# NyanCAD/Cadnip.jl

Hardware: AMD Instinct MI355X
Metric: newton_iters_per_sec (higher is better)
Workload: dtype f64; 1 GPU; gf180 DFF transient 0-700 ns (synthetic sp_mos1 level-1 card, 30 MOSFETs, n=235, nnz=1090), 4096 Vdd x temp corner instances per GPU (state resident in HBM; one 8-instance workgroup per CU in flight, the rest handed out by the kernel's instance queue); step = DC init + full transient of the batch; instances_per_gpu=4096, instances_total=4096, fused=2, newton_mode=1, launches_last_step=5120, accepted_last_step=6078488, rejected_last_step=692364

## Files before the change

### cadnip.jl_amd/csrc/devices.hpp

```cpp
#pragma once
#include <hip/hip_runtime.h>
#include <math.h>
#include "../../include/cadnip_hip.h"

namespace cadnip {

#define CADNIP_CHARGE_SCALE 1e12

#ifdef CADNIP_TRACE
static __device__ unsigned long long g_trace_sum[64], g_trace_cnt[64];
static __device__ int g_trace_wave;
__shared__ unsigned long long g_trace_last;
#define CADNIP_TRACE_FINE(id) (((id) >= 8 && (id) <= 15) || (id) >= 18 || (id) == 0 || (id) == 2)
#define CADNIP_TRACE_POINT(id)                                                                          \
  do {                                                                                                  \
    if ((CADNIP_TRACE + 0 >= 2 || !CADNIP_TRACE_FINE(id)) && blockIdx.x == 0 && (int)(threadIdx.x >> 6) == g_trace_wave) { \
      unsigned long long _t = clock64();                                                                \
      if ((threadIdx.x & 63) == 0) {                                                                    \
        atomicAdd(&g_trace_sum[id], _t - g_trace_last); atomicAdd(&g_trace_cnt[id], 1ull); g_trace_last = _t; \
      }                                                                                                 \
    }                                                                                                   \
  } while (0)
#define CADNIP_TRACE_USE(x) asm volatile("" ::"v"(x))
#elif defined(CADNIP_MARKS)
#define CADNIP_TRACE_POINT(id) asm volatile("; @@MARK " #id)
#define CADNIP_TRACE_USE(x) do {} while (0)
#else
#define CADNIP_TRACE_POINT(id) do {} while (0)
#define CADNIP_TRACE_USE(x) do {} while (0)
#endif

__device__ __forceinline__ double dpp_pair_swap(double v) {
  int lo = __double2loint(v), hi = __double2hiint(v);
  lo = __builtin_amdgcn_update_dpp(0, lo, 0xB1, 0xF, 0xF, false);
  hi = __builtin_amdgcn_update_dpp(0, hi, 0xB1, 0xF, 0xF, false);
  return __hiloint2double(hi, lo);
}

template <class NodeT> struct DevCtxT {
  const NodeT* __restrict__ nodes;
  const int* __restrict__ ipar;
  const double* __restrict__ par;
  const double* __restrict__ wave;
  int count;
// ... 525 lines not shown
  {
    const bool fwd = o_vds >= 0;
    const double q_vgs = fwd ? vgs : vgd + (vgs - vgd), q_vgd = fwd ? vgs - (vgs - vgd) : vgd, q_vds = vgs - vgd;
    const bool c1 = fabs(fwd ? vgs - o_vgs : vgd - vgdo) <= 0.4, c2 = fabs(q_vds - o_vds) <= 0.4;
    const bool c3 = q_vds >= 0 ? !(fabs(vbs - o_vbs) > (vt + vt)) : !(fabs(vbd - o_vbd) > (vt + vt));
    if (__all(c1 && c2 && c3)) {
      double r_vgs = q_vgs, r_vds = q_vds, r_vbs, r_vbd;
      (void)q_vgd;
      if (r_vds >= 0) { r_vbs = vbs; r_vbd = r_vbs - r_vds; }
      else { r_vbd = vbd; r_vbs = r_vbd + r_vds; }
      if (d.initjct) { r_vbs = -1; r_vgs = type * par_of(d, M1_TVTO); r_vds = 0; r_vbd = r_vbs - r_vds; }
      w_gs = type * r_vgs; w_ds = type * r_vds; w_bs = type * r_vbs; w_bd = type * r_vbd;
      return;
    }
  }
  int omode = o_vds >= 0 ? 1 : -1;
  double osel = omode == 1 ? o_vbs : o_vbd, osarg;
  if (osel <= 0) osarg = sqrt(tPhi - osel);
  else { osarg = sqrt(tPhi); osarg = osarg - o_vbs / (osarg + osarg); osarg = fmax(0.0, osarg); }
  double o_von = (tVbi * type) + gamma * osarg;
  double von = type * o_von;
  if (o_vds >= 0) {
    vgs = m1_fetlim(vgs, o_vgs, von);
    vds = vgs - vgd;
    vds = m1_limvds(vds, o_vds);
    vgd = vgs - vds;
  } else {
    vgd = m1_fetlim(vgd, vgdo, von);
    vds = vgs - vgd;
    vds = -m1_limvds(-vds, -o_vds);
// ... 466 lines not shown
```

### cadnip.jl_amd/csrc/fused2_kernel.hpp

```cpp
#pragma once
#include <hip/hip_runtime.h>
#include "devices.hpp"
#include "internal.hpp"
#include "tran_ctrl.hpp"
#include "lds_layout.hpp"
#include "src_cache.hpp"

namespace cadnip {

typedef unsigned short u16;
typedef unsigned long long u64;
#define NOPOS 0xFFFFu
#define F2_NCMAX 16
#define F2_JU 18
#define F2_MAX_BLOCKS 32

enum { S_GPOS = 0, S_CDESC, S_BROW, S_NZ, S_ENT, S_TERM, S_LEV, S_QINV, S_NODES, S_ROWOF, S_LOADPOS, S_NSEC };

struct F2Block {
  const int* ipar; const double* par;
  int type, count, n_par, g_base, c_base, b_base, nodes_off, mos1_plain;
  int lds_par;
};

// ... 85 lines not shown
    atomicAdd(&W[tg(gpos[k * count + dev])], v);
  }
  __device__ __forceinline__ void C(int k, double v) const {
    if (!JAC) return;
    if (__builtin_constant_p(v) && v == 0.0) return;
    const u64 d = cdesc[k * count + dev];
    atomicAdd(&W[tg((unsigned)d & 0xFFFFu)], a0 * v);
    if (!DIRECT) atomicAdd(&W[tg((unsigned)(d >> 16) & 0xFFFFu)], v * betas[(unsigned)(d >> 32) & 0xFFFFu]);
  }
  __device__ __forceinline__ void B(int k, double v) const {
    if (DIRECT || (__builtin_constant_p(v) && v == 0.0)) return;
    atomicAdd(&W[tg(brow[k * count + dev])], -v);
  }
  template <int N> __device__ __forceinline__ void Gv(int k0, const double (&v)[N]) const {
    if (!JAC) return;
    unsigned p[N];
#pragma unroll
    for (int i = 0; i < N; ++i) p[i] = gpos[(k0 + i) * count + dev];
#pragma unroll
    for (int i = 0; i < N; ++i) if (!(__builtin_constant_p(v[i]) && v[i] == 0.0)) atomicAdd(&W[tg(p[i])], v[i]);
  }
  template <int N> __device__ __forceinline__ void Gk(const int (&k)[N], const double (&v)[N]) const {
    if (!JAC) return;
    unsigned p[N];
#pragma unroll
    for (int i = 0; i < N; ++i) p[i] = gpos[k[i] * count + dev];
#pragma unroll
    for (int i = 0; i < N; ++i) atomicAdd(&W[tg(p[i])], v[i]);
  }
  template <int N> __device__ __forceinline__ void Cv(int k0, const double (&v)[N]) const {
// ... 14 lines not shown
      }
  }
  template <int N> __device__ __forceinline__ void Bv(int k0, const double (&v)[N]) const {
    if (DIRECT) return;
    unsigned p[N];
#pragma unroll
    for (int i = 0; i < N; ++i) p[i] = brow[(k0 + i) * count + dev];
#pragma unroll
    for (int i = 0; i < N; ++i) if (!(__builtin_constant_p(v[i]) && v[i] == 0.0)) atomicAdd(&W[tg(p[i])], -v[i]);
  }
};

typedef DevCtxT<short> LdsCtx;

struct F2M1ParMem {
  int bi, inst, dev;
  __device__ __forceinline__ double operator()(int k) const {
    const F2ArgsK ka = kargs();
    const F2Block B = load_block(ka->blk, bi);
    return (B.par + (size_t)inst * B.n_par * B.count)[k * B.count + dev];
  }
};

template <bool LEAN, class Out>
__device__ __forceinline__ void dispatch_stamp2(int type, const LdsCtx& d, const double* u, const Out& s, double* lw) {
  if constexpr (LEAN) {
    switch (type) {
      case CADNIP_DEV_RESISTOR: stamp_resistor(d, u, s, lw); break;
      case CADNIP_DEV_CAPACITOR: stamp_capacitor(d, u, s, lw); break;
      case CADNIP_DEV_INDUCTOR: stamp_inductor(d, u, s, lw); break;
      case CADNIP_DEV_VSOURCE: stamp_vsource(d, u, s, lw); break;
      case CADNIP_DEV_ISOURCE: stamp_isource(d, u, s, lw); break;
      case CADNIP_DEV_VCVS: stamp_vcvs(d, u, s, lw); break;
      case CADNIP_DEV_VCCS: stamp_vccs(d, u, s, lw); break;
// ... 83 lines not shown
  __device__ __forceinline__ double h3(int i, int) const { return (kargs()->t.u3 + vo)[i]; }
  __device__ __forceinline__ void set_h3(int i, int, double v) { (kargs()->t.u3 + vo)[i] = v; }
  __device__ __forceinline__ void set_h0(int i, int k, double v) { if (k >= 0) r_u0[k] = v; else p_u0()[i] = v; }
  __device__ __forceinline__ void set_h1(int i, int k, double v) { if (k >= 0) r_u1[k] = v; else p_u1()[i] = v; }
  __device__ __forceinline__ void set_h2(int i, int k, double v) { if (k >= 0) r_u2[k] = v; else p_u2()[i] = v; }
  __device__ __forceinline__ void set_hp(int i, int k, double v) { if (k >= 0) r_up[k] = v; else p_up()[i] = v; }
  __device__ __forceinline__ double atol_of(const TranArgs& a, int i, int k) const { return k >= 0 ? pf_at[k] : a.atol[i]; }
  __device__ __forceinline__ double emask_of(const TranArgs& a, int i, int k) const { return k >= 0 ? pf_em[k] : a.emask[i]; }
};

template <int NC, int MODE>
__device__ __forceinline__ void dense_core_solve(double* W, int dn0, int yc0, int lane, int& bad, bool keep) {
  const int row = lane < NC ? lane : 0;
  double* S = W + dn0 + row * NC;
  double A[NC], rp[NC], bc = W[yc0 + row];
#pragma unroll
  for (int j = 0; j < NC; ++j) A[j] = S[j];
#pragma unroll
  for (int k = 0; k < NC; ++k) {
    const double pkk = readlane_f64(A[k], k);
    if (MODE == 0 && (pkk == 0.0 || !isfinite(pkk))) bad = 1;
    rp[k] = MODE == 0 ? fast_div(1.0, pkk) : pkk;
    const double m = lane > k ? (MODE == 0 ? A[k] * rp[k] : A[k]) : 0.0;
    if (MODE == 0) {
#pragma unroll
      for (int j = k + 1; j < NC; ++j) A[j] = fma(-m, readlane_f64(A[j], k), A[j]);
      if (lane > k) A[k] = m;
    }
    bc = fma(-m, readlane_f64(bc, k), bc);
  }
// ... 41 lines not shown
      const uint4* src = (const uint4*)f.team_desc;
      uint4* dst = (uint4*)L.desc;
      unsigned char* fl = (unsigned char*)(L.desc + f.team_desc_len);
      for (int i = tid; i < f.team_desc_len / 2; i += 64 * WPB) {
        const uint4 d = src[i];
        const StepPredec p = lds_step_predecode(d.x, d.y, d.z, d.w, (unsigned)(f.nnz_lu + n + lane0));
        dst[i] = make_uint4(p.x, p.y, p.z, p.w);
        fl[i] = (unsigned char)p.flags;
      }
    } else {
      const uint2* src = (const uint2*)f.team_desc;
      uint2* dst = (uint2*)L.desc;
      for (int i = tid; i < f.team_desc_len; i += 64 * WPB) dst[i] = src[i];
    }
  }
  __syncthreads();
  const int nW = L.nW;
  double* W = L.W;
  double* us = L.u;
  double* betas = L.beta;
  if (lane0 == 0) { W[nW] = 0.0; W[nW + 1] = 1.0; }
  const int tlo = f.tab_lo;
  const u16* gpos = (const u16*)(tab + (f.off[S_GPOS] - tlo));
  const u64* cdesc = (const u64*)(tab + (f.off[S_CDESC] - tlo));
  const u16* brow = (const u16*)(tab + (f.off[S_BROW] - tlo));
  const u64* nzd = (const u64*)(tab + (LEAN ? 0 : f.off[S_NZ]));
  const u64* laned = (const u64*)(tab + (LEAN ? 0 : f.off[S_ENT]));
  const unsigned* term = tab + (LEAN ? 0 : f.off[S_TERM]);
  typedef const __attribute__((address_space(4))) u64* PassPtr;
  const PassPtr passd = (PassPtr)(const u64*)(f.tab + f.off[S_LEV]);
  const u16* qinv = (const u16*)(tab + (f.off[S_QINV] - tlo));
  const short* nodes = (const short*)(tab + (f.off[S_NODES] - tlo));
  const u16* rowof = (const u16*)(tab + (f.off[S_ROWOF] - tlo));
  unsigned rc_gp[RCQ][2] = {}, rc_row[RCQ] = {}, rc_nd[RCQ] = {}, src_gp[2] = {0, 0}, src_row[2] = {0, 0}, src_nd[2] = {0, 0};
  int rc_count = 0, rc_type = 0, src_count = 0, src_type = 0;
  M1PairView<F2M1ParMem> m1v;
  if constexpr (DIRECT) {
    const unsigned tr = (unsigned)(f.nnz_lu + n + lane0);
    auto row_of = [&](int node) -> unsigned { return node < 0 ? tr : (unsigned)rowof[node]; };
    if (SHAPE ? true : f.rc_blk >= 0) {
      const F2Block B = load_block(f.blk, f.rc_blk);
      rc_count = B.count; rc_type = B.type;
      const short* nd = nodes + B.nodes_off;
#pragma unroll
      for (int q = 0; q < RCQ; ++q) {
        const int dev = lane0 + 64 * q;
        unsigned p[4] = {tr, tr, tr, tr};
        int np = -1, nn = -1;
        if (dev < B.count) {
          np = nd[dev]; nn = nd[B.count + dev];
#pragma unroll
// ... 10 lines not shown
      src_count = B.count; src_type = B.type;
      const short* nd = nodes + B.nodes_off;
      unsigned p[4] = {tr, tr, tr, tr};
      int np = -1, nn = -1, ni = -1;
      if (lane0 < B.count) {
        np = nd[lane0]; nn = nd[B.count + lane0];
        if (SHAPE ? true : B.type == CADNIP_DEV_VSOURCE) {
          ni = nd[2 * B.count + lane0];
#pragma unroll
          for (int k = 0; k < 4; ++k) p[k] = (unsigned)gpos[B.g_base + k * B.count + lane0];
        }
      }
      src_gp[0] = p[0] | p[1] << 16; src_gp[1] = p[2] | p[3] << 16;
      src_row[0] = row_of(np) | row_of(nn) << 16; src_row[1] = row_of(ni);
      src_nd[0] = ((unsigned)np & 0xFFFFu) | ((unsigned)nn & 0xFFFFu) << 16; src_nd[1] = (unsigned)ni & 0xFFFFu;
    }
    if constexpr (SHAPE) {
      const F2Block B = load_block(f.blk, 3 - f.rc_blk - f.src_blk);
      const short* nd = nodes + B.nodes_off;
      const int dv = lane0 >> 1, dev = dv < B.count ? dv : B.count - 1, sd = lane0 & 1;
      const int vdep = B.ipar[dev];
      auto node = [&](int k) -> int { return nd[k * B.count + dev]; };
      auto qnode = [&](int r) -> int { return ((vdep >> r) & 1) ? node(10 + r) : -1; };
      auto opd2 = [&](int na, int nb) -> unsigned { return lds_m1pin_operand(na, f.nnz_lu, n) | lds_m1pin_operand(nb, f.nnz_lu, n) << 16; };
      auto row2 = [&](int na, int nb) -> unsigned { return lds_m1pin_row(rowof, na, tr) | lds_m1pin_row(rowof, nb, tr) << 16; };
#pragma unroll
      for (int j = 0; j < 5; ++j) m1v.opd[j] = opd2(node(2 * j), node(2 * j + 1));
      m1v.opd[5] = opd2(qnode(sd), qnode(2 + sd));
      m1v.row[0] = sd ? row2(node(8), node(9)) : row2(node(6), node(7));
      m1v.row[1] = row2(sd ? node(4) : node(3), node(5));
      m1v.row[2] = row2(qnode(sd), sd ? node(3) : node(1));
      m1v.row[3] = row2(qnode(2 + sd), sd ? node(5) : node(4));
      m1v.initjct = 0;
      m1v.gnd = lds_m1pin_operand(-1, f.nnz_lu, n); m1v.beta = 8u * (unsigned)n;
    }
  }
#ifdef CADNIP_TRACE
  if (blockIdx.x == 0 && tid == 0) g_trace_last = clock64();
#endif
  int inst = blockIdx.x * WPB + w;
  int budget = f.rounds;
  for (;;) {
  StepState st;
  bool have = false;
  while (inst < f.B) {
    const TranStateView sv = state_view<FIXED>();
    if (DC) st.status = __builtin_amdgcn_readfirstlane(sv.status[inst]);
    else { st = load_state(sv, inst); make_uniform(st); }
// ... 42 lines not shown
  double src_val = 0.0, src_t = 0.0;
  bool src_have = false;
  int src_seg = 0;
  for (; budget > 0; --budget) {
    int lane = lane0;
    asm volatile("" : "+v"(lane));
    CADNIP_TRACE_POINT(17);
    bool refresh = true;
    if (mn) {
      refresh = (st.mflags & MN_NEED) || !(st.mflags & MN_VALID) ||
                (st.k == 0 && (st.a0 < 0.6 * st.a0f || st.a0 * 0.6 > st.a0f || (st.mflags >> MN_SINCE_SHIFT) >= 20));
      if (refresh) { st.a0f = st.a0; st.ss = 20.0; st.mflags = MN_VALID | MN_JCUR; st.dsc = 1.0; }
      else st.dsc = st.a0 == st.a0f ? 1.0 : fast_div(2.0, 1.0 + fast_div(st.a0, st.a0f));
    }
    if (refresh) {
      for (int i = lane; i < (nW >> 1); i += 64) ((double2*)W)[i] = make_double2(0.0, 0.0);
    } else if constexpr (FIXED) {
#pragma unroll
      for (int k = 0; k < 5; ++k) { const int i = f.nnz_lu + lane + 64 * k; if (i < nW) W[i] = 0.0; }
    } else {
      for (int i = f.nnz_lu + lane; i < nW; i += 64) W[i] = 0.0;
    }
    CADNIP_WAVE_SYNC();
    CADNIP_TRACE_POINT(0);
    const double tcur = DC ? 0.0 : st.tn, a0 = DC ? 0.0 : st.a0;
    const int dmode = DC ? f.dc_mode : 1, dinit = DC ? dc_first : 0;
    const unsigned trash_w = (unsigned)(f.nnz_lu + n + lane);
    dc_first = 0;
    if constexpr (DIRECT) {
      auto at = [&](unsigned nd16) -> double { const double x = us[nd16 == 0xFFFFu ? 0u : nd16]; return nd16 == 0xFFFFu ? 0.0 : x; };
// ... 4 lines not shown
      };
      if (SHAPE ? true : f.rc_blk >= 0) {
        const bool cap = SHAPE ? true : rc_type == CADNIP_DEV_CAPACITOR;
        double jv[RCQ], cur[RCQ];
#pragma unroll
        for (int q = 0; q < RCQ; ++q) {
          const unsigned np = rc_nd[q] & 0xFFFFu, nn = rc_nd[q] >> 16;
          const double xp = cap ? dat(np) : at(np), xn = cap ? dat(nn) : at(nn);
          jv[q] = cap ? a0 * rc_val[q] : rc_val[q];
          cur[q] = rc_val[q] * (xp - xn);
        }
#pragma unroll
        for (int q = 0; q < RCQ; ++q) {
          if (q == 1 && rc_count <= 64) break;
          if (refresh) {
            atomicAdd(&W[rc_gp[q][0] & 0xFFFFu], jv[q]); atomicAdd(&W[rc_gp[q][0] >> 16], -jv[q]);
            atomicAdd(&W[rc_gp[q][1] & 0xFFFFu], -jv[q]); atomicAdd(&W[rc_gp[q][1] >> 16], jv[q]);
          }
          atomicAdd(&W[rc_row[q] & 0xFFFFu], cur[q]); atomicAdd(&W[rc_row[q] >> 16], -cur[q]);
        }
      }
      CADNIP_TRACE_POINT(14);
      if (SHAPE ? true : f.src_blk >= 0) {
        if (DC || !src_have || tcur != src_t) {
          const int cl = src_cache_lanes(src_count);
          const bool sc = sc_on();
          int miss = 1;
          double cv = 0.0;
          if (sc) {
            const SrcSeg e = src_seg_load((const double*)L.src, cl, lane < cl ? lane : 0);
            miss = src_seg_hit(e, tcur) ? 0 : 1;
            cv = src_seg_value(e, tcur);
          }
          if (wave_any(miss)) {
            const F2Block B = load_block(f.blk, f.src_blk);
            const double* par = B.par + (size_t)inst * B.n_par * B.count;
            LdsCtx d{nodes + B.nodes_off, B.ipar, par, f.wave, B.count, lane < B.count ? lane : 0, tcur, dmode, dinit};
            src_val = source_value(d, par_of(d, 0), par_of(d, 1), &src_seg);
          } else src_val = cv;
          if (sc_on() && miss && lane < cl) {
            const F2ArgsK ka = kargs();
            const F2Block B = load_block(ka->blk, ka->src_blk);
            SrcSeg r = src_seg_never();
            if (B.ipar[lane] == 1) {
              const int len = B.ipar[2 * B.count + lane];
              const double* wv = ka->wave + B.ipar[B.count + lane];
              r = src_seg_refill(1, wv, wv + len, len, src_seg, (B.par + (size_t)inst * B.n_par * B.count)[B.count + lane]);
            }
            src_seg_store(L.src, cl, lane, r);
          }
          src_t = tcur; src_have = true;
        }
        CADNIP_TRACE_USE(src_val);
        CADNIP_TRACE_POINT(15);
        if (SHAPE ? true : src_type == CADNIP_DEV_VSOURCE) {
          const double ui = at(src_nd[1]), vd = at(src_nd[0] & 0xFFFFu) - at(src_nd[0] >> 16) - src_val;
          if (refresh) {
            atomicAdd(&W[src_gp[0] & 0xFFFFu], 1.0); atomicAdd(&W[src_gp[0] >> 16], -1.0);
            atomicAdd(&W[src_gp[1] & 0xFFFFu], 1.0); atomicAdd(&W[src_gp[1] >> 16], -1.0);
          }
          atomicAdd(&W[src_row[0] & 0xFFFFu], ui); atomicAdd(&W[src_row[0] >> 16], -ui);
          atomicAdd(&W[src_row[1]], vd);
        } else {
          atomicAdd(&W[src_row[0] & 0xFFFFu], -src_val); atomicAdd(&W[src_row[0] >> 16], src_val);
        }
      }
      CADNIP_TRACE_POINT(13);
    }
    if constexpr (SHAPE) {
      const int bi = 3 - f.rc_blk - f.src_blk;
      const F2Block B = load_block(f.blk, bi);
      const int side = lane & 1;
      const int dv = lane >> 1;
      const bool valid = dv < B.count;
      const int dev = valid ? dv : B.count - 1;
#pragma unroll
      for (int j = 0; j < 6; ++j) asm volatile("" : "+v"(m1v.opd[j]));
#pragma unroll
      for (int j = 0; j < 4; ++j) asm volatile("" : "+v"(m1v.row[j]));
      m1_pair_each_param(m1v, [](double& x) { asm volatile("" : "+v"(x)); });
      m1v.W = W; m1v.mem = F2M1ParMem{bi, inst, dev};
      if (!refresh) {
        AccumOutT<true, DIRECT, false> s{W, betas, a0, gpos + B.g_base, cdesc + B.c_base, brow + B.b_base, B.count, dev, valid ? 0u : trash_w, us, rowof, trash_w};
        stamp_mos1_pair(m1v, us, s, lw, side, valid);
      } else {
        AccumOutT<true, DIRECT> s{W, betas, a0, gpos + B.g_base, cdesc + B.c_base, brow + B.b_base, B.count, dev, valid ? 0u : trash_w, us, rowof, trash_w};
        stamp_mos1_pair(m1v, us, s, lw, side, valid);
      }
      CADNIP_TRACE_POINT(8);
    }
    if constexpr (!SHAPE)
    for (int bi = 0; bi < f.n_blk; ++bi) {
      if (DIRECT && ((bi == f.rc_blk && rc_count <= 128) || (bi == f.src_blk && src_count <= 64))) continue;
      const F2Block B = load_block(f.blk, bi);
      const double* par = B.par + (size_t)inst * B.n_par * B.count;
      int dev0 = lane;
      if (DIRECT && bi == f.rc_blk) dev0 = lane + 128;
      if (DIRECT && bi == f.src_blk) dev0 = lane + 64;
      if (!DIRECT && bi == f.rc_blk) {
#pragma unroll
        for (int q = 0; q < 2; ++q) {
// ... 159 lines not shown
        double part = fma(a2v, b2v, fma(a1v, b1v, a0v * b0v));
        if (maxlg >= 1) { const double o = dpp_f64<0xB1>(part); part += lg >= 1 ? o : 0.0; }
        if (maxlg >= 2) { const double o = dpp_f64<0x4E>(part); part += lg >= 2 ? o : 0.0; }
        if (maxlg >= 3) { const double o = dpp_f64<0x141>(part); part += lg >= 3 ? o : 0.0; }
        if (maxlg >= 4) { const double o = dpp_f64<0x140>(part); part += lg >= 4 ? o : 0.0; }
        double acc = acc0 - part;
        if (fw >> 31) {
          if (piv == 0.0 || !isfinite(piv)) bad = 1;
          acc = fast_div(acc, piv);
        }
        *((D.x & 0x8000u) ? pp : W + trash_w) = acc;
        D = Dn;
      }
      CADNIP_WAVE_SYNC();
    };
    auto run_steps_pd = [&](const int s_first, const int s_count) {
      if (s_count <= 0) return;
      const uint4* dp = tdesc + (size_t)s_first * 64 + lane;
      const unsigned char* fp = tflag + (size_t)s_first * 64 + lane;
      char* const Wb = (char*)W;
      uint4 D = dp[0];
      unsigned F = fp[0];
      for (int si = 0; si < s_count; ++si) {
        double* const pp = (double*)(Wb + (D.x & 0xFFFFu));
        const double piv = *(const double*)(Wb + (D.x >> 16));
        const double a0v = *(const double*)(Wb + (D.y & 0xFFFFu)), b0v = *(const double*)(Wb + (D.y >> 16));
        const double a1v = *(const double*)(Wb + (D.z & 0xFFFFu)), b1v = *(const double*)(Wb + (D.z >> 16));
        const double a2v = *(const double*)(Wb + (D.w & 0xFFFFu)), b2v = *(const double*)(Wb + (D.w >> 16));
        const double acc0 = *pp;
        const uint4 Dn = dp[(size_t)(si + 1) * 64];
        const unsigned Fn = fp[(size_t)(si + 1) * 64];
        const unsigned fs = __builtin_amdgcn_readfirstlane(F), maxlg = fs & 7u;
        double part = fma(a2v, b2v, fma(a1v, b1v, a0v * b0v));
        if (maxlg >= 1) { const double o = dpp_f64<0xB1>(part); part += F >= 16u ? o : 0.0; }
        if (maxlg >= 2) { const double o = dpp_f64<0x4E>(part); part += F >= 32u ? o : 0.0; }
        if (maxlg >= 3) { const double o = dpp_f64<0x141>(part); part += F >= 48u ? o : 0.0; }
        if (maxlg >= 4) { const double o = dpp_f64<0x140>(part); part += F >= 64u ? o : 0.0; }
        double acc = acc0 - part;
        if (fs & 8u) {
          if (piv == 0.0 || !isfinite(piv)) bad = 1;
          acc = fast_div(acc, piv);
        }
        *pp = acc;
        D = Dn; F = Fn;
      }
      CADNIP_WAVE_SYNC();
    };
    auto solve_steps = [&](const int s_first, const int s_count) {
      if (predec) run_steps_pd(s_first, s_count); else run_steps(s_first, s_count);
    };
    if constexpr (LEAN) {
      solve_steps(refresh ? 0 : f.ts_pre + f.ts_post, refresh ? f.ts_pre : f.ts_fwd);
    } else {
      if (refresh) run_passes(0, f.n_pre);
      else run_passes(f.n_pre + f.n_post, f.n_fwd);
    }
    CADNIP_TRACE_POINT(4);
    if constexpr (FIXED) {
      const int yc0 = f.nnz_lu + n - 8;
      if (refresh) dense_core_solve<8, 0>(W, f.dn0, yc0, lane, bad, true);
      else dense_core_solve<8, 1>(W, f.dn0, yc0, lane, bad, false);
      CADNIP_WAVE_SYNC();
    } else if (f.nc > 0) {
      const int yc0 = f.nnz_lu + n - f.nc;
      if (refresh) DENSE_CORE(0, f.nc, W, f.dn0, yc0, lane, bad, mn);
      else if (LEAN && !DC) DENSE_CORE(1, f.nc, W, f.dn0, yc0, lane, bad, false);
      CADNIP_WAVE_SYNC();
    }
    CADNIP_TRACE_POINT(5);
    if constexpr (LEAN) solve_steps(f.ts_pre, f.ts_post); else run_passes(f.n_pre, f.n_post);
    CADNIP_TRACE_POINT(3);
    if (DC) {
      for (int i = lane; i < n; i += 64) { const double dd = W[qinv[i]]; if (!isfinite(dd)) bad = 1; us[i] -= dd; }
      bad = wave_any(bad);
      CADNIP_WAVE_SYNC();
      if (f.dc_pcnr && a.n_limits > 0) {
        __builtin_amdgcn_fence(__ATOMIC_ACQ_REL, "workgroup");
        for (int i = n - a.n_limits + lane; i < n; i += 64) us[i] = lw[i];
      }
      if (bad) st.status = -2; else dc_iters += 1;
    } else {
      tran_update_body(a, vec, st, inst, lane, bad);
      make_uniform(st);
    }
    CADNIP_WAVE_SYNC();
// ... 50 lines not shown
```

### cadnip.jl_amd/csrc/lds_layout.hpp

```cpp
#pragma once
#include <stddef.h>
#include "../../include/cadnip_hip.h"
#ifdef __HIPCC__
#include <type_traits>
#define LDS_HD __host__ __device__ __forceinline__
#else
#define LDS_HD inline
#endif

#define F2_TRASH 64
#define LDS_BUDGET ((size_t)160 * 1024)
#define LDS_OPTIN ((size_t)64 * 1024)

namespace cadnip {

LDS_HD int lds_work_words(int lu_words, int n) { return lu_words + n + F2_TRASH; }
#define LDS_CONSTS 2

struct StepPredec { unsigned x, y, z, w, flags; };
LDS_HD StepPredec lds_step_predecode(unsigned x, unsigned y, unsigned z, unsigned w, unsigned trash_word) {
  StepPredec r;
  r.x = ((x & 0x8000u) ? (x & 0x7FFFu) : trash_word) << 3 | ((x >> 16) & 0x7FFFu) << 19;
  r.y = (y & 0x7FFF7FFFu) << 3; r.z = (z & 0x7FFF7FFFu) << 3; r.w = (w & 0x7FFF7FFFu) << 3;
  const unsigned lg = (x >> 31) | ((y >> 14) & 2u) | ((y >> 29) & 4u);
// ... 6 lines not shown
                        int use_pcnr, bool enabled) {
  return tran && lean && newton_mode == 1 && step_predec && src_words > 0 && n <= 256 && nc == 8 && max_order <= 2 && step_rule == 0 &&
         use_pcnr == 0 && enabled;
}
LDS_HD bool f2_shape_ok(bool fixed, int n_blk, int src_type, int src_count, int rc_type, int rc_count, int dev_type, int dev_plain, int dev_count,
                        bool enabled) {
  return fixed && n_blk == 3 && src_type == CADNIP_DEV_VSOURCE && src_count <= 64 && rc_type == CADNIP_DEV_CAPACITOR && rc_count <= 64 &&
         dev_type == CADNIP_DEV_MOS1 && dev_plain != 0 && dev_count <= 32 && enabled;
}
LDS_HD bool lds_m1pin_ok(int lu_words, int n) { return lds_work_words(lu_words, n) + LDS_CONSTS + n <= 8192; }
LDS_HD unsigned lds_m1pin_operand(int node, int lu_words, int n) {
  const int nW = lds_work_words(lu_words, n);
  return (unsigned)(node < 0 ? nW : nW + LDS_CONSTS + node) << 3;
}
template <class T> LDS_HD unsigned lds_m1pin_row(const T* rowof, int node, unsigned trash_word) { return node < 0 ? trash_word : (unsigned)rowof[node]; }
LDS_HD int lds_sweep_desc_words(int desc_len, bool predec) { return desc_len + (predec ? desc_len / 16 : 0); }

template <class P> struct LdsSweep { P desc, W, u, beta, end; int nW, per; P src; };
template <class P> LDS_HD LdsSweep<P> lds_sweep(P base, int tab_len, int desc_len, int lu_words, int n, int w, int wpb, int src_words = 0) {
  LdsSweep<P> L;
  L.nW = lds_work_words(lu_words, n);
  L.per = L.nW + LDS_CONSTS + 2 * n + src_words;
  L.desc = base + tab_len / 2;
  L.W = L.desc + desc_len + (size_t)w * L.per;
  L.u = L.W + L.nW + LDS_CONSTS; L.beta = L.u + n; L.src = L.beta + n;
  L.end = L.desc + desc_len + (size_t)wpb * L.per;
  return L;
}

template <class P> struct LdsTeam { P W, red, u, beta, par, desc, priv, end; int nW; };
// ... 56 lines not shown
```

### cadnip.jl_amd/csrc/tran_ctrl.hpp

```cpp
#pragma once
#include <hip/hip_runtime.h>
#include <math.h>

namespace cadnip {

#define CADNIP_WAVE_SYNC() do { __builtin_amdgcn_fence(__ATOMIC_ACQ_REL, "wavefront"); __builtin_amdgcn_wave_barrier(); } while (0)

template <int CTRL> __device__ __forceinline__ double dpp_f64(double v) {
  int lo = __double2loint(v), hi = __double2hiint(v);
  lo = __builtin_amdgcn_update_dpp(0, lo, CTRL, 0xF, 0xF, true);
  hi = __builtin_amdgcn_update_dpp(0, hi, CTRL, 0xF, 0xF, true);
  return __hiloint2double(hi, lo);
}
__device__ __forceinline__ double group_sum16(double v, int width) {
  if (width >= 2) v += dpp_f64<0xB1>(v);
  if (width >= 4) v += dpp_f64<0x4E>(v);
  if (width >= 8) v += dpp_f64<0x141>(v);
  if (width >= 16) v += dpp_f64<0x140>(v);
  return v;
}
__device__ __forceinline__ double readlane_f64(double v, int l) {
  return __hiloint2double(__builtin_amdgcn_readlane(__double2hiint(v), l), __builtin_amdgcn_readlane(__double2loint(v), l));
}
__device__ __forceinline__ double wave_sum(double v) {
// ... 16 lines not shown
  int e;
  double m = frexp(x, &e);
  const int q = (e >= 0 ? e : e - 2) / 3;
  m = ldexp(m, e - 3 * q);
  double y = fma(m, -0.17, 1.18);
#pragma unroll
  for (int it = 0; it < 4; ++it) {
    const double y3 = (y * y) * y;
    y = (y * fma(-m, y3, 4.0)) * (1.0 / 3.0);
  }
  return ldexp(y, -q);
}

#ifndef CADNIP_TRACE_POINT
#define CADNIP_TRACE_POINT(id) do {} while (0)
#endif
struct TranArgs {
  double *u, *du, *delta, *limit_w, *tcur, *gamma;
  int *active, *flags;
  double *t, *h, *hprev, *hpp; int *nhist, *order, *k, *status, *bp_idx, *save_idx; long long* cnt;
  double *u0, *u1, *u2, *up, *beta;
  const double *atol, *emask, *breaks, *save_t; const int* obs; double* out; int* nactive;
  int B, n, n_limits, n_break, n_save, n_obs, n_err;
  double t0, t1, reltol, h0, hmin, hmax, newton_tol;
  int max_newton, max_order, use_pcnr;
  int newton_mode;
  double *mn_a0f, *mn_ss, *mn_dnp; int* mn_flags;
  int step_rule;
  double *u3, *hp3;
};
// ... 142 lines not shown
  }
}

template <class V>
__device__ inline void prepare_step(const TranArgs& a, V& v, StepState& s, int tid, double t, double h, int nhist, double hprev, double hpp) {
  const int n = a.n;
  double tstop = a.t1;
  if (s.t_break < tstop) tstop = s.t_break;
  double rem = tstop - t, tn;
  if (h >= rem * (1.0 - 1e-9)) { h = rem; tn = tstop; }
  else if (2.0 * h > rem) { h = 0.5 * rem; tn = t + h; }
  else tn = t + h;
  int ord;
  double a0;
  if (nhist <= 1) {
    ord = 1; a0 = fast_div(1.0, h);
    each_elem<V>(n, tid, [&](int i, int k) { double p = v.h0(i, k); v.set_hp(i, k, p); v.set_u(i, p); double b = fast_div(-p, h); v.set_beta(i, b); v.set_du(i, a0 * p + b); });
  } else if (nhist == 2 || a.max_order < 2) {
    ord = 1; a0 = fast_div(1.0, h);
    double w = fast_div(h, hprev);
    each_elem<V>(n, tid, [&](int i, int k) {
      double x0 = v.h0(i, k);
      double p = x0 + w * (x0 - v.h1(i, k));
      v.set_hp(i, k, p); v.set_u(i, p);
      double b = fast_div(-x0, h);
      v.set_beta(i, b); v.set_du(i, a0 * p + b);
    });
  } else if (nhist >= 4 && (!V::FIXED && a.max_order >= 3)) {
    ord = 3;
    const double hr = s.hp3;
    const double d1 = h, d2 = h + hprev, d3 = d2 + hpp, s12 = hprev + hpp;
    a0 = (fast_div(1.0, d1) + fast_div(1.0, d2)) + fast_div(1.0, d3);
    const double a1 = -fast_div(d2 * d3, d1 * (hprev * s12)), a2 = fast_div(d1 * d3, d2 * (hprev * hpp)), a3 = -fast_div(d1 * d2, d3 * (s12 * hpp));
// ... 22 lines not shown
      double x0 = v.h0(i, k), xm1 = v.h1(i, k);
      double p = L0 * x0 + L1 * xm1 + L2 * v.h2(i, k);
      v.set_hp(i, k, p); v.set_u(i, p);
      double b = a1 * x0 + a2 * xm1;
      v.set_beta(i, b); v.set_du(i, a0 * p + b);
    });
  }
  s.h = h; s.ord = ord; s.k = 0; s.tn = tn; s.a0 = a0;
  s.mflags &= ~MN_JCUR;
}

template <class V>
__device__ inline void save_outputs(const TranArgs& a, V& v, StepState& s, int inst, int tid) {
  const double told = s.t, tn = s.tn, hh = tn - told;
  int si = s.si;
  if (s.t_save <= tn * (1.0 + 1e-15)) v.history_to_memory(a.n, tid);
  while (s.t_save <= tn * (1.0 + 1e-15)) {
    double ts = s.t_save;
    double* o = a.out + ((size_t)inst * a.n_save + si) * a.n_obs;
    if (s.nhist >= 2) {
      double x = ts - told, xa = hh, xc = -s.hprev;
      double La = fast_div((x - 0.0) * (x - xc), (xa - 0.0) * (xa - xc));
      double Lb = fast_div((x - xa) * (x - xc), (0.0 - xa) * (0.0 - xc));
      double Lc = fast_div((x - xa) * (x - 0.0), (xc - xa) * (xc - 0.0));
      for (int j = tid; j < a.n_obs; j += V::NT) { int i = a.obs[j]; o[j] = La * v.get_u(i) + Lb * v.mem_u0(i) + Lc * v.mem_u1(i); }
    } else {
      double sc = fast_div(ts - told, hh);
      for (int j = tid; j < a.n_obs; j += V::NT) { int i = a.obs[j]; double x0 = v.mem_u0(i); o[j] = x0 + sc * (v.get_u(i) - x0); }
    }
    ++si;
    s.t_save = next_save(a, si);
  }
// ... 58 lines not shown
      const int nh_cap = (!V::FIXED && a.max_order >= 3) ? 4 : 3;
      int nh_new = s.nhist + 1 > nh_cap ? nh_cap : s.nhist + 1;
      double hnext;
      if (tested) {
        double fac;
        if (V::FIXED || a.step_rule == 0) {
          fac = errn > 0.0 ? 0.9 * step_root(errn, (V::FIXED ? (s.ord == 1 ? 1 : 2) : s.ord)) : 2.0;
          fac = fmin(2.0, fmax(0.2, fac));
        } else {
          const double eta = errn > 0.0 ? fast_div(1.0, fast_div(1.0, step_root(2.0 * errn, (V::FIXED ? (s.ord == 1 ? 1 : 2) : s.ord))) + 1e-4) : 2.0;
          fac = eta >= 2.0 ? 2.0 : (eta <= 1.0 ? fmax(0.5, fmin(0.9, eta)) : 1.0);
        }
        hnext = h * fac;
      } else hnext = 2.0 * h;
      if (landed) {
        ++s.bp;
        s.t_break = next_break(a, s.bp);
        nh_new = 1;
        double tstop = a.t1;
        if (s.t_break < tstop) tstop = s.t_break;
        hnext = 0.1 * fmin(h, tstop - tn);
      }
      hnext = fmin(hnext, a.hmax);
      s.hp3 = hpp;
      s.t = tn; s.hpp = hprev; s.hprev = h; s.nhist = nh_new;
      s.c_accept += 1;
      s.mflags += 1 << MN_SINCE_SHIFT;
      CADNIP_TRACE_POINT(31);
      if (tn >= a.t1) { s.status = 1; return; }
      if (hnext < a.hmin) hnext = a.hmin;
      grp_sync<V>();
      prepare_step(a, v, s, tid, tn, hnext, nh_new, s.hprev, s.hpp);
      CADNIP_TRACE_POINT(32);
    } else {
      double fac;
      if (V::FIXED || a.step_rule == 0) { fac = 0.9 * step_root(errn, (V::FIXED ? (s.ord == 1 ? 1 : 2) : s.ord)); fac = fmin(0.9, fmax(0.1, fac)); }
      else { fac = fast_div(0.9, fast_div(1.0, step_root(2.0 * errn, (V::FIXED ? (s.ord == 1 ? 1 : 2) : s.ord))) + 1e-4); fac = fmin(0.9, fmax(0.25, fac)); }
      double hn = h * fac;
      s.c_reject += 1;
      if (hn < a.hmin) { s.status = -1; return; }
      grp_sync<V>();
      prepare_step(a, v, s, tid, s.t, hn, s.nhist, hprev, hpp);
    }
  } else {
    if ((V::FIXED || a.newton_mode) && (bad || diverge || s.k + 1 >= a.max_newton) && !(s.mflags & MN_JCUR)) {
      s.mflags |= MN_NEED;
      grp_sync<V>();
      prepare_step(a, v, s, tid, s.t, h, s.nhist, hprev, hpp);
    } else if (bad || diverge || s.k + 1 >= a.max_newton) {
      double hn = 0.25 * h;
      s.c_fail += 1;
      if (hn < a.hmin) { s.status = -2; return; }
      grp_sync<V>();
      prepare_step(a, v, s, tid, s.t, hn, s.nhist, hprev, hpp);
    } else {
      grp_sync<V>();
      if (!V::FIXED && a.use_pcnr && a.n_limits > 0)
        for (int i = n - a.n_limits + tid; i < n; i += V::NT) v.set_u(i, v.get_lw(i));
      grp_sync<V>();
      const double a0 = s.a0;
      if constexpr (!V::FIXED) for (int i = tid; i < n; i += V::NT) v.set_du(i, a0 * v.get_u(i) + v.get_beta(i));
      s.k += 1;
    }
  }
// ... 4 lines not shown
```

Before: 186.5 million newton_iters/s.

## Cache MOS1 block scalars and step-table LDS addresses in SGPRs, add rare-path markers

The MOS1 pair block's count and base offsets are now hoisted out of the Newton loop and pinned in scalar registers, so the block descriptor is no longer reloaded every iteration. In the non-refresh path the gpos/cdesc/brow pointers are passed as null. The shaped solve computes packed LDS addresses and step counts for the triangular step tables once and reads descriptors from LDS. Source node reads use precomputed byte offsets, and assembly marker macros are added on rare paths for profiling. Together these aim to cut scalar and address overhead in the hot loop, at the cost of extra SGPR pressure and reliance on the packed-count bit limits.

```diff
diff --git a/cadnip.jl_amd/csrc/devices.hpp b/cadnip.jl_amd/csrc/devices.hpp
--- a/cadnip.jl_amd/csrc/devices.hpp
+++ b/cadnip.jl_amd/csrc/devices.hpp
@@ -28,6 +28,11 @@
 #else
 #define CADNIP_TRACE_POINT(id) do {} while (0)
 #define CADNIP_TRACE_USE(x) do {} while (0)
+#endif
+#ifdef CADNIP_MARKS
+#define CADNIP_RARE_POINT(id) asm volatile("; @@RARE " #id)
+#else
+#define CADNIP_RARE_POINT(id) do {} while (0)
 #endif
 
 __device__ __forceinline__ double dpp_pair_swap(double v) {
@@ -583,6 +588,7 @@
       return;
     }
   }
+  CADNIP_RARE_POINT(48);
   int omode = o_vds >= 0 ? 1 : -1;
   double osel = omode == 1 ? o_vbs : o_vbd, osarg;
   if (osel <= 0) osarg = sqrt(tPhi - osel);
diff --git a/cadnip.jl_amd/csrc/fused2_kernel.hpp b/cadnip.jl_amd/csrc/fused2_kernel.hpp
--- a/cadnip.jl_amd/csrc/fused2_kernel.hpp
+++ b/cadnip.jl_amd/csrc/fused2_kernel.hpp
@@ -123,6 +123,7 @@
   }
   template <int N> __device__ __forceinline__ void Gv(int k0, const double (&v)[N]) const {
     if (!JAC) return;
+    if constexpr (GUARD) CADNIP_RARE_POINT(46);
     unsigned p[N];
 #pragma unroll
     for (int i = 0; i < N; ++i) p[i] = gpos[(k0 + i) * count + dev];
@@ -167,10 +168,10 @@
 typedef DevCtxT<short> LdsCtx;
 
 struct F2M1ParMem {
-  int bi, inst, dev;
+  int inst, dev;
   __device__ __forceinline__ double operator()(int k) const {
     const F2ArgsK ka = kargs();
-    const F2Block B = load_block(ka->blk, bi);
+    const F2Block B = load_block(ka->blk, 3 - ka->rc_blk - ka->src_blk);
     return (B.par + (size_t)inst * B.n_par * B.count)[k * B.count + dev];
   }
 };
@@ -284,6 +285,7 @@
   const int row = lane < NC ? lane : 0;
   double* S = W + dn0 + row * NC;
   double A[NC], rp[NC], bc = W[yc0 + row];
+  if (MODE == 0) CADNIP_RARE_POINT(47);
 #pragma unroll
   for (int j = 0; j < NC; ++j) A[j] = S[j];
 #pragma unroll
@@ -355,6 +357,7 @@
       for (int i = tid; i < f.team_desc_len; i += 64 * WPB) dst[i] = src[i];
     }
   }
+  const unsigned sp_addr = SHAPE ? lds_steps_pack_addr(f.tab_len, f.team_desc_len) : 0u, sp_cnt = SHAPE ? lds_steps_pack_counts(f.ts_pre, f.ts_post, f.ts_fwd) : 0u;
   __syncthreads();
   const int nW = L.nW;
   double* W = L.W;
@@ -376,6 +379,7 @@
   unsigned rc_gp[RCQ][2] = {}, rc_row[RCQ] = {}, rc_nd[RCQ] = {}, src_gp[2] = {0, 0}, src_row[2] = {0, 0}, src_nd[2] = {0, 0};
   int rc_count = 0, rc_type = 0, src_count = 0, src_type = 0;
   M1PairView<F2M1ParMem> m1v;
+  int m1_count = 0, m1_gbase = 0, m1_cbase = 0;
   if constexpr (DIRECT) {
     const unsigned tr = (unsigned)(f.nnz_lu + n + lane0);
     auto row_of = [&](int node) -> unsigned { return node < 0 ? tr : (unsigned)rowof[node]; };
@@ -416,6 +420,9 @@
       src_gp[0] = p[0] | p[1] << 16; src_gp[1] = p[2] | p[3] << 16;
       src_row[0] = row_of(np) | row_of(nn) << 16; src_row[1] = row_of(ni);
       src_nd[0] = ((unsigned)np & 0xFFFFu) | ((unsigned)nn & 0xFFFFu) << 16; src_nd[1] = (unsigned)ni & 0xFFFFu;
+      if constexpr (SHAPE) {
+        src_nd[0] = lds_m1pin_operand(np, f.nnz_lu, n) | lds_m1pin_operand(nn, f.nnz_lu, n) << 16; src_nd[1] = lds_m1pin_operand(ni, f.nnz_lu, n);
+      }
     }
     if constexpr (SHAPE) {
       const F2Block B = load_block(f.blk, 3 - f.rc_blk - f.src_blk);
@@ -434,6 +441,8 @@
       m1v.row[2] = row2(qnode(sd), sd ? node(3) : node(1));
       m1v.row[3] = row2(qnode(2 + sd), sd ? node(5) : node(4));
       m1v.initjct = 0;
+      m1_count = B.count; m1_gbase = B.g_base; m1_cbase = B.c_base;
+      asm volatile("" : "+s"(m1_count), "+s"(m1_gbase), "+s"(m1_cbase));
       m1v.gnd = lds_m1pin_operand(-1, f.nnz_lu, n); m1v.beta = 8u * (unsigned)n;
     }
   }
@@ -506,6 +515,7 @@
       else st.dsc = st.a0 == st.a0f ? 1.0 : fast_div(2.0, 1.0 + fast_div(st.a0, st.a0f));
     }
     if (refresh) {
+      CADNIP_RARE_POINT(41);
       for (int i = lane; i < (nW >> 1); i += 64) ((double2*)W)[i] = make_double2(0.0, 0.0);
     } else if constexpr (FIXED) {
 #pragma unroll
@@ -540,6 +550,7 @@
         for (int q = 0; q < RCQ; ++q) {
           if (q == 1 && rc_count <= 64) break;
           if (refresh) {
+            CADNIP_RARE_POINT(42);
             atomicAdd(&W[rc_gp[q][0] & 0xFFFFu], jv[q]); atomicAdd(&W[rc_gp[q][0] >> 16], -jv[q]);
             atomicAdd(&W[rc_gp[q][1] & 0xFFFFu], -jv[q]); atomicAdd(&W[rc_gp[q][1] >> 16], jv[q]);
           }
@@ -559,12 +570,14 @@
             cv = src_seg_value(e, tcur);
           }
           if (wave_any(miss)) {
+            CADNIP_RARE_POINT(43);
             const F2Block B = load_block(f.blk, f.src_blk);
             const double* par = B.par + (size_t)inst * B.n_par * B.count;
             LdsCtx d{nodes + B.nodes_off, B.ipar, par, f.wave, B.count, lane < B.count ? lane : 0, tcur, dmode, dinit};
             src_val = source_value(d, par_of(d, 0), par_of(d, 1), &src_seg);
           } else src_val = cv;
           if (sc_on() && miss && lane < cl) {
+            CADNIP_RARE_POINT(44);
             const F2ArgsK ka = kargs();
             const F2Block B = load_block(ka->blk, ka->src_blk);
             SrcSeg r = src_seg_never();
@@ -580,8 +593,11 @@
         CADNIP_TRACE_USE(src_val);
         CADNIP_TRACE_POINT(15);
         if (SHAPE ? true : src_type == CADNIP_DEV_VSOURCE) {
-          const double ui = at(src_nd[1]), vd = at(src_nd[0] & 0xFFFFu) - at(src_nd[0] >> 16) - src_val;
+          auto atw = [&](unsigned off) -> double { return *(const double*)((const char*)W + off); };
+          const double ui = SHAPE ? atw(src_nd[1]) : at(src_nd[1]);
+          const double vd = (SHAPE ? atw(src_nd[0] & 0xFFFFu) : at(src_nd[0] & 0xFFFFu)) - (SHAPE ? atw(src_nd[0] >> 16) : at(src_nd[0] >> 16)) - src_val;
           if (refresh) {
+            CADNIP_RARE_POINT(45);
             atomicAdd(&W[src_gp[0] & 0xFFFFu], 1.0); atomicAdd(&W[src_gp[0] >> 16], -1.0);
             atomicAdd(&W[src_gp[1] & 0xFFFFu], 1.0); atomicAdd(&W[src_gp[1] >> 16], -1.0);
           }
@@ -594,23 +610,22 @@
       CADNIP_TRACE_POINT(13);
     }
     if constexpr (SHAPE) {
-      const int bi = 3 - f.rc_blk - f.src_blk;
-      const F2Block B = load_block(f.blk, bi);
+      asm volatile("" : "+s"(m1_count));
       const int side = lane & 1;
       const int dv = lane >> 1;
-      const bool valid = dv < B.count;
-      const int dev = valid ? dv : B.count - 1;
+      const bool valid = dv < m1_count;
+      const int dev = valid ? dv : m1_count - 1;
 #pragma unroll
       for (int j = 0; j < 6; ++j) asm volatile("" : "+v"(m1v.opd[j]));
 #pragma unroll
       for (int j = 0; j < 4; ++j) asm volatile("" : "+v"(m1v.row[j]));
       m1_pair_each_param(m1v, [](double& x) { asm volatile("" : "+v"(x)); });
-      m1v.W = W; m1v.mem = F2M1ParMem{bi, inst, dev};
+      m1v.W = W; m1v.mem = F2M1ParMem{inst, dev};
       if (!refresh) {
-        AccumOutT<true, DIRECT, false> s{W, betas, a0, gpos + B.g_base, cdesc + B.c_base, brow + B.b_base, B.count, dev, valid ? 0u : trash_w, us, rowof, trash_w};
+        AccumOutT<true, DIRECT, false> s{W, betas, a0, nullptr, nullptr, nullptr, m1_count, dev, valid ? 0u : trash_w, us, rowof, trash_w};
         stamp_mos1_pair(m1v, us, s, lw, side, valid);
       } else {
-        AccumOutT<true, DIRECT> s{W, betas, a0, gpos + B.g_base, cdesc + B.c_base, brow + B.b_base, B.count, dev, valid ? 0u : trash_w, us, rowof, trash_w};
+        AccumOutT<true, DIRECT> s{W, betas, a0, gpos + m1_gbase, cdesc + m1_cbase, nullptr, m1_count, dev, valid ? 0u : trash_w, us, rowof, trash_w};
         stamp_mos1_pair(m1v, us, s, lw, side, valid);
       }
       CADNIP_TRACE_POINT(8);
@@ -800,10 +815,10 @@
       }
       CADNIP_WAVE_SYNC();
     };
-    auto run_steps_pd = [&](const int s_first, const int s_count) {
+    auto run_steps_pd = [&](const uint4* const td, const unsigned char* const tf, const int s_first, const int s_count) {
       if (s_count <= 0) return;
-      const uint4* dp = tdesc + (size_t)s_first * 64 + lane;
-      const unsigned char* fp = tflag + (size_t)s_first * 64 + lane;
+      const uint4* dp = td + (size_t)s_first * 64 + lane;
+      const unsigned char* fp = tf + (size_t)s_first * 64 + lane;
       char* const Wb = (char*)W;
       uint4 D = dp[0];
       unsigned F = fp[0];
@@ -833,9 +848,19 @@
       CADNIP_WAVE_SYNC();
     };
     auto solve_steps = [&](const int s_first, const int s_count) {
-      if (predec) run_steps_pd(s_first, s_count); else run_steps(s_first, s_count);
+      if (predec) run_steps_pd(tdesc, tflag, s_first, s_count); else run_steps(s_first, s_count);
     };
-    if constexpr (LEAN) {
+    auto sp_steps = [&](const int which) {
+      unsigned pa = sp_addr, pc = sp_cnt;
+      asm volatile("" : "+s"(pa), "+s"(pc));
+      const int pre = lds_steps_pack_pre(pc), post = lds_steps_pack_post(pc), fwd = lds_steps_pack_fwd(pc);
+      const uint4* const td = (const uint4*)((const char*)sm + lds_steps_pack_desc(pa));
+      const unsigned char* const tf = (const unsigned char*)sm + lds_steps_pack_flag(pa);
+      if (which == 0) run_steps_pd(td, tf, refresh ? 0 : pre + post, refresh ? pre : fwd);
+      else run_steps_pd(td, tf, pre, post);
+    };
+    if constexpr (SHAPE) sp_steps(0);
+    else if constexpr (LEAN) {
       solve_steps(refresh ? 0 : f.ts_pre + f.ts_post, refresh ? f.ts_pre : f.ts_fwd);
     } else {
       if (refresh) run_passes(0, f.n_pre);
@@ -854,7 +879,8 @@
       CADNIP_WAVE_SYNC();
     }
     CADNIP_TRACE_POINT(5);
-    if constexpr (LEAN) solve_steps(f.ts_pre, f.ts_post); else run_passes(f.n_pre, f.n_post);
+    if constexpr (SHAPE) sp_steps(1);
+    else if constexpr (LEAN) solve_steps(f.ts_pre, f.ts_post); else run_passes(f.n_pre, f.n_post);
     CADNIP_TRACE_POINT(3);
     if (DC) {
       for (int i = lane; i < n; i += 64) { const double dd = W[qinv[i]]; if (!isfinite(dd)) bad = 1; us[i] -= dd; }
diff --git a/cadnip.jl_amd/csrc/lds_layout.hpp b/cadnip.jl_amd/csrc/lds_layout.hpp
--- a/cadnip.jl_amd/csrc/lds_layout.hpp
+++ b/cadnip.jl_amd/csrc/lds_layout.hpp
@@ -44,6 +44,16 @@
   return (unsigned)(node < 0 ? nW : nW + LDS_CONSTS + node) << 3;
 }
 template <class T> LDS_HD unsigned lds_m1pin_row(const T* rowof, int node, unsigned trash_word) { return node < 0 ? trash_word : (unsigned)rowof[node]; }
+LDS_HD unsigned lds_steps_pack_addr(int tab_len, int desc_len) {
+  const unsigned desc_b = (unsigned)tab_len * 4u, flag_b = desc_b + (unsigned)desc_len * 8u;
+  return desc_b >> 4 | (flag_b >> 4) << 16;
+}
+LDS_HD unsigned lds_steps_pack_desc(unsigned addr) { return (addr & 0xFFFFu) << 4; }
+LDS_HD unsigned lds_steps_pack_flag(unsigned addr) { return (addr >> 16) << 4; }
+LDS_HD unsigned lds_steps_pack_counts(int pre, int post, int fwd) { return (unsigned)pre | (unsigned)post << 10 | (unsigned)fwd << 20; }
+LDS_HD int lds_steps_pack_pre(unsigned c) { return (int)(c & 1023u); }
+LDS_HD int lds_steps_pack_post(unsigned c) { return (int)((c >> 10) & 1023u); }
+LDS_HD int lds_steps_pack_fwd(unsigned c) { return (int)(c >> 20); }
 LDS_HD int lds_sweep_desc_words(int desc_len, bool predec) { return desc_len + (predec ? desc_len / 16 : 0); }
 
 template <class P> struct LdsSweep { P desc, W, u, beta, end; int nW, per; P src; };
diff --git a/cadnip.jl_amd/csrc/tran_ctrl.hpp b/cadnip.jl_amd/csrc/tran_ctrl.hpp
--- a/cadnip.jl_amd/csrc/tran_ctrl.hpp
+++ b/cadnip.jl_amd/csrc/tran_ctrl.hpp
@@ -54,6 +54,9 @@
 
 #ifndef CADNIP_TRACE_POINT
 #define CADNIP_TRACE_POINT(id) do {} while (0)
+#endif
+#ifndef CADNIP_RARE_POINT
+#define CADNIP_RARE_POINT(id) do {} while (0)
 #endif
 struct TranArgs {
   double *u, *du, *delta, *limit_w, *tcur, *gamma;
@@ -226,9 +229,11 @@
   int ord;
   double a0;
   if (nhist <= 1) {
+    CADNIP_RARE_POINT(56);
     ord = 1; a0 = fast_div(1.0, h);
     each_elem<V>(n, tid, [&](int i, int k) { double p = v.h0(i, k); v.set_hp(i, k, p); v.set_u(i, p); double b = fast_div(-p, h); v.set_beta(i, b); v.set_du(i, a0 * p + b); });
   } else if (nhist == 2 || a.max_order < 2) {
+    CADNIP_RARE_POINT(57);
     ord = 1; a0 = fast_div(1.0, h);
     double w = fast_div(h, hprev);
     each_elem<V>(n, tid, [&](int i, int k) {
@@ -281,8 +286,9 @@
 __device__ inline void save_outputs(const TranArgs& a, V& v, StepState& s, int inst, int tid) {
   const double told = s.t, tn = s.tn, hh = tn - told;
   int si = s.si;
-  if (s.t_save <= tn * (1.0 + 1e-15)) v.history_to_memory(a.n, tid);
+  if (s.t_save <= tn * (1.0 + 1e-15)) { CADNIP_RARE_POINT(54); v.history_to_memory(a.n, tid); }
   while (s.t_save <= tn * (1.0 + 1e-15)) {
+    CADNIP_RARE_POINT(54);
     double ts = s.t_save;
     double* o = a.out + ((size_t)inst * a.n_save + si) * a.n_obs;
     if (s.nhist >= 2) {
@@ -371,6 +377,7 @@
         hnext = h * fac;
       } else hnext = 2.0 * h;
       if (landed) {
+        CADNIP_RARE_POINT(55);
         ++s.bp;
         s.t_break = next_break(a, s.bp);
         nh_new = 1;
@@ -384,12 +391,13 @@
       s.c_accept += 1;
       s.mflags += 1 << MN_SINCE_SHIFT;
       CADNIP_TRACE_POINT(31);
-      if (tn >= a.t1) { s.status = 1; return; }
+      if (tn >= a.t1) { CADNIP_RARE_POINT(58); s.status = 1; return; }
       if (hnext < a.hmin) hnext = a.hmin;
       grp_sync<V>();
       prepare_step(a, v, s, tid, tn, hnext, nh_new, s.hprev, s.hpp);
       CADNIP_TRACE_POINT(32);
     } else {
+      CADNIP_RARE_POINT(51);
       double fac;
       if (V::FIXED || a.step_rule == 0) { fac = 0.9 * step_root(errn, (V::FIXED ? (s.ord == 1 ? 1 : 2) : s.ord)); fac = fmin(0.9, fmax(0.1, fac)); }
       else { fac = fast_div(0.9, fast_div(1.0, step_root(2.0 * errn, (V::FIXED ? (s.ord == 1 ? 1 : 2) : s.ord))) + 1e-4); fac = fmin(0.9, fmax(0.25, fac)); }
@@ -401,10 +409,12 @@
     }
   } else {
     if ((V::FIXED || a.newton_mode) && (bad || diverge || s.k + 1 >= a.max_newton) && !(s.mflags & MN_JCUR)) {
+      CADNIP_RARE_POINT(52);
       s.mflags |= MN_NEED;
       grp_sync<V>();
       prepare_step(a, v, s, tid, s.t, h, s.nhist, hprev, hpp);
     } else if (bad || diverge || s.k + 1 >= a.max_newton) {
+      CADNIP_RARE_POINT(53);
       double hn = 0.25 * h;
       s.c_fail += 1;
       if (hn < a.hmin) { s.status = -2; return; }
```

Result: no change. 188.0 million newton_iters/s (median of 4 runs) (+0.8%).
